# Emieeel/auto_oo

Hardware: AMD Instinct MI355X
Metric: OO-VQE energy+grad evals/sec (formaldimine CAS(4e,3o)/cc-pVDZ); 2e-transform fp64 TFLOP/s vs roofline (higher is better)
Workload: dtype f64; 1 GPU; configs[1] shape: N=43 AOs, n_occ=6, CAS(4e,3o), UCCD n_theta=4, n_kappa=327; one step = one batched call evaluating energy + full gradient of all 256 geometries of the rank (256 synthetic geometries in the job, geometry g on rank g mod n_gpus); value = evaluations/s; in-order calls on one stream; geometries_per_rank=256, batched_calls=1332, calls=in order, parallelism=geometry-sharded x1, one all_gather at the end, dist_world_size=1, devices_visible=1, device_of_rank0=0

## Files before the change

### auto_oo_amd/csrc/cas.hip

```cpp
#include "plan.h"
#include "circuit_small.h"
#include <type_traits>
#include <stdlib.h>

namespace {

constexpr int HALF_WAVES = 8;
constexpr int TRI_REG_R = 3;
constexpr int tiles_depth(int zt) { return zt == 3 ? 4 : 8; }
constexpr int stream_depth(int zt) { return zt == 3 ? 2 : 3; }
constexpr int AUX_PLAIN = 0, AUX_NT = 2;

constexpr int SYM_FULL = 0, SYM_MIRROR = 1, SYM_PACKED = 2;
__device__ __forceinline__ void tri_decode(long t, int N, int& p, int& q)
{
    const double b = 2.0 * N + 1.0;
    int pp = (int)((b - sqrt(b * b - 8.0 * (double)t)) * 0.5);
    pp = pp < 0 ? 0 : (pp > N - 1 ? N - 1 : pp);
    while (pp > 0 && (long)pp * (2 * N - pp + 1) / 2 > t) --pp;
    while (pp < N - 1 && (long)(pp + 1) * (2 * N - pp) / 2 <= t) ++pp;
    p = pp;
    q = pp + (int)(t - (long)pp * (2 * N - pp + 1) / 2);
}

// ... 2312 lines not shown
                      const int32_t* __restrict__ kap_row, const int32_t* __restrict__ kap_col,
                      int n_kappa, double* __restrict__ c0, double* __restrict__ E,
                      double* __restrict__ gvec, double* __restrict__ dE, double* __restrict__ fock,
                      double* __restrict__ gmat, const double* __restrict__ nuc_arr,
                      size_t out_stride)
{
    const int tid = threadIdx.x;
    {
        const size_t gi = blockIdx.x;
        Fcol += gi * (size_t)nrdm * M * N;
        Epart += gi * (size_t)nrdm * N;
        Cpart += gi * (size_t)N;
        c0 += gi * out_stride;
        E += gi * out_stride;
        gvec += gi * out_stride;
        if (dE) dE += gi * out_stride;
        if (fock) fock += gi * (size_t)N * N;
        if (gmat) gmat += gi * (size_t)N * N;
        if (nuc_arr) nuc = nuc_arr[gi];
    }
    for (long base = 0; base < (long)nrdm * n_kappa; base += 4 * 512) {
        int rr[4], cc[4], kk[4];
#pragma unroll
        for (int u = 0; u < 4; ++u) {
            const long idx = base + u * 512 + tid;
            const bool ok = idx < (long)nrdm * n_kappa;
            const long ii = ok ? idx : 0;
            kk[u] = (int)(ii / n_kappa);
            const int t = (int)(ii - (long)kk[u] * n_kappa);
            rr[u] = kap_row[t];
            cc[u] = kap_col[t];
        }
        double frc[4], fcr[4];
#pragma unroll
        for (int u = 0; u < 4; ++u) {
            const double* F = Fcol + (size_t)kk[u] * M * N;
            const int r = rr[u], c = cc[u];
            frc[u] = F[(size_t)(r < M ? r : 0) * N + c] * (r < M ? 1.0 : 0.0);
            fcr[u] = F[(size_t)(c < M ? c : 0) * N + r] * (c < M ? 1.0 : 0.0);
        }
#pragma unroll
        for (int u = 0; u < 4; ++u) {
            const long idx = base + u * 512 + tid;
            if (idx < (long)nrdm * n_kappa) gvec[idx] = 2.0 * (frc[u] - fcr[u]);
        }
    }
    if (fock)
        for (int idx = tid; idx < N * N; idx += 512) {
            const int m = idx / N;
            fock[idx] = m < M ? Fcol[idx] : 0.0;
        }
    if (gmat)
        for (int idx = tid; idx < N * N; idx += 512) {
            const int m = idx / N, n = idx - m * N;
            const double fmn = m < M ? Fcol[(size_t)m * N + n] : 0.0;
            const double fnm = n < M ? Fcol[(size_t)n * N + m] : 0.0;
            gmat[idx] = 2.0 * (fmn - fnm);
        }
    if (tid < nrdm) {
        const int k = tid;
        double acc = 0.0;
        for (int n = 0; n < M; ++n) acc += Epart[(size_t)k * N + n];
        if (k == 0) {
            double core = nuc;
            for (int n = 0; n < M; ++n) core += Cpart[n];
            c0[0] = core;
            E[0] = core + acc;
        } else if (dE) {
            dE[k - 1] = acc;
        }
    }
}

constexpr int TAIL_THREADS = 512;

__host__ __device__ inline bool tail_needed(int x, int y, int z, int no)
{
    const int lo = y < z ? y : z, hi = y < z ? z : y;
    if (lo >= no) return true;
    if (hi < no) return lo == hi || x == lo || x == hi;
    return x >= no || x == lo;
}

template <int KS>
__global__ __launch_bounds__(TAIL_THREADS, 2)
void cas_tail_kernel(const double* __restrict__ J, const double* __restrict__ C, const double* __restrict__ Wpre,
                     const double* __restrict__ gamma, const double* __restrict__ Gamma, int nrdm, int N, int no,
                     int na, int NC, double nuc, const double* __restrict__ nuc_arr,
                     const int32_t* __restrict__ kap_row, const int32_t* __restrict__ kap_col, int n_kappa,
                     double* __restrict__ c0, double* __restrict__ E, double* __restrict__ gvec,
                     double* __restrict__ dE, double* __restrict__ c1, double* __restrict__ c2, size_t out_stride)
{
    extern __shared__ double lds[];
    constexpr int NW = TAIL_THREADS / 64;
    constexpr int PW = (4 * KS + NW - 1) / NW;
    constexpr int PB = PW * KS > 48 ? (PW + 1) / 2 : PW;
    const int M = no + na, M2 = M * M, M3 = M2 * M;
    const int na2 = na * na, na3 = na2 * na, na4 = na2 * na2;
    const int ncol = M * (M + 1) / 2, nty = (ncol + 15) / 16;
    const long tri = (long)N * (N + 1) / 2;
    const int by = blockIdx.x;
    const int tid = threadIdx.x, lane = tid & 63;
    const int wave = __builtin_amdgcn_readfirstlane(tid >> 6);
    const int lq = lane >> 4, lr = lane & 15;
    {
        const size_t gi = by;
        J += gi * nty * tri * 16;
        C += gi * (size_t)N * N;
        Wpre += gi * (size_t)N * N;
        gamma += gi * (size_t)nrdm * na2;
        Gamma += gi * (size_t)nrdm * na4;
        c0 += gi * out_stride;
        E += gi * out_stride;
        gvec += gi * out_stride;
        if (dE) dE += gi * out_stride;
        c1 += gi * out_stride;
        c2 += gi * out_stride;
        if (nuc_arr) nuc = nuc_arr[gi];
    }
    double* Gc = lds;
    double* Cl = Gc + (size_t)N * NC;
    double* hn = Cl + (size_t)N * M;
    double* FIn = hn + (size_t)N * M;
    double* gml = FIn + (size_t)N * M;
    double* Gml = gml + (size_t)nrdm * na2;
    double* Cp = Gml + (size_t)nrdm * na4;
    int* tab = reinterpret_cast<int*>(Cp + N);
    int* wcnt = tab + M3;
    int* krow = wcnt + NW;
    int* kcol = krow + n_kappa;
    double* scr = Cp + N + (M3 + NW + 2 * n_kappa + 1) / 2;
    const int LDP = M * 16 + 8;

    typedef unsigned v2u __attribute__((ext_vector_type(2)));
    const __amdgpu_buffer_rsrc_t csrd = __builtin_amdgcn_make_buffer_rsrc(
        const_cast<double*>(C), 0, (int)((size_t)N * N * sizeof(double)), 0x00020000);
    double af[KS];
#pragma unroll
    for (int ks = 0; ks < KS; ++ks) {
        const int q = 4 * ks + lq;
        const v2u v = __builtin_amdgcn_raw_buffer_load_b64(
            csrd, (q < N && lr < M) ? (unsigned)((q * N + lr) * (int)sizeof(double)) : 0x7fffffffu, 0, 0);
        af[ks] = __builtin_bit_cast(double, v);
    }
    auto load_half = [&](double (&bf)[PB][KS], int ty, int h0) {
        const __amdgpu_buffer_rsrc_t jsrd = __builtin_amdgcn_make_buffer_rsrc(
            const_cast<double*>(J + (size_t)ty * tri * 16), 0, (int)(tri * 16 * sizeof(double)), 0x00020000);
#pragma unroll
        for (int i = 0; i < PB; ++i) {
            const int p = wave + NW * (h0 + i);
            const int pc = p < N ? p : N - 1;
            const int basep = pc * (2 * N - pc + 1) / 2 - pc;
#pragma unroll
            for (int ks = 0; ks < KS; ++ks) {
                const int q = 4 * ks + lq < N ? 4 * ks + lq : N - 1;
                const int t = q < pc ? q * (2 * N - q + 1) / 2 - q + pc : basep + q;
                const v2u v = __builtin_amdgcn_raw_buffer_load_b64(
                    jsrd, (unsigned)((t * 16 + lr) * (int)sizeof(double)), 0, 0);
                bf[i][ks] = __builtin_bit_cast(double, v);
            }
        }
    };
    double* T3s = scr;
    auto mfma_half = [&](const double (&bf)[PB][KS], int h0) {
#pragma unroll
        for (int i = 0; i < PB; ++i) {
            if (h0 + i >= PW) continue;
            const int p = wave + NW * (h0 + i);
            d4 acc = d4{0.0, 0.0, 0.0, 0.0};
#pragma unroll
            for (int ks = 0; ks < KS; ++ks) acc = mfma_f64(af[ks], bf[i][ks], acc);
            double* row = T3s + (size_t)(p < 4 * KS ? p : 0) * LDP + lr;
#pragma unroll
            for (int j = 0; j < 4; ++j) {
                const int x = lq + 4 * j;
                if (x < M && p < 4 * KS) row[x * 16] = p < N ? acc[j] : 0.0;
            }
        }
    };
    static_assert(2 * PB >= PW, "two halves cover the rows of a wave");
    double bf[PB][KS];
    load_half(bf, 0, 0);

    for (int idx = tid; idx < N * M; idx += TAIL_THREADS) {
        const int q = idx / M, x = idx - q * M;
        Cl[idx] = C[(size_t)q * N + x];
    }
    for (int idx = tid; idx < N * N; idx += TAIL_THREADS) scr[idx] = Wpre[idx];
    for (int idx = tid; idx < nrdm * na2; idx += TAIL_THREADS) gml[idx] = gamma[idx];
    for (int idx = tid; idx < nrdm * na4; idx += TAIL_THREADS) Gml[idx] = Gamma[idx];
    for (int idx = tid; idx < n_kappa; idx += TAIL_THREADS) {
        krow[idx] = kap_row[idx];
        kcol[idx] = kap_col[idx];
    }
    {
        const int total = M * ncol;
        int base = 0;
        for (int i0 = 0; i0 < total; i0 += TAIL_THREADS) {
            const int i = i0 + tid;
            int x = 0, y = 0, z = 0;
            bool need = false;
            if (i < total) {
                x = i / ncol;
                tri_decode(i - x * ncol, M, y, z);
                need = tail_needed(x, y, z, no);
            }
            const unsigned long long mask = __ballot(need);
            const int below = __popcll(mask & ((1ull << lane) - 1ull));
            if (lane == 0) wcnt[wave] = __popcll(mask);
            __syncthreads();
            int pre = base, all = 0;
            for (int w = 0; w < NW; ++w) {
                const int c = wcnt[w];
                if (w < wave) pre += c;
                all += c;
            }
            if (i < total) {
                const int v = need ? pre + below : -1;
                tab[(x * M + y) * M + z] = v;
                tab[(x * M + z) * M + y] = v;
            }
            __syncthreads();
            base += all;
        }
    }
    for (int idx = tid; idx < N * M; idx += TAIL_THREADS) {
        const int n = idx / M, x = idx - n * M;
        double acc = 0.0;
        for (int q = 0; q < N; ++q) acc += scr[(size_t)n * N + q] * Cl[q * M + x];
        hn[idx] = acc;
    }
    __syncthreads();

    {
        const int ntn = (N + 15) / 16;
        for (int ty = 0; ty < nty; ++ty) {
            mfma_half(bf, 0);
            if (PB < PW) {
                load_half(bf, ty, PB);
                mfma_half(bf, PB);
            }
            __syncthreads();
            const int yz = 16 * ty + lr;
            int off = 0;
            if (yz < ncol) {
                int y, z;
                tri_decode(yz, M, y, z);
                off = y * M + z;
            }
            int cur_nt = -1;
            double cf[KS];
            for (int tile = wave; tile < ntn * M; tile += NW) {
                const int nt = tile / M, x = tile - nt * M;
                if (nt != cur_nt) {
                    const int n = 16 * nt + lr;
#pragma unroll
                    for (int ks = 0; ks < KS; ++ks) {
                        const int pp = 4 * ks + lq;
                        const v2u v = __builtin_amdgcn_raw_buffer_load_b64(
                            csrd, (pp < N && n < N) ? (unsigned)((pp * N + n) * (int)sizeof(double)) : 0x7fffffffu,
                            0, 0);
                        cf[ks] = __builtin_bit_cast(double, v);
                    }
                    cur_nt = nt;
                }
                double tf[KS];
#pragma unroll
                for (int ks = 0; ks < KS; ++ks) tf[ks] = T3s[(size_t)(4 * ks + lq) * LDP + x * 16 + lr];
                d4 acc = d4{0.0, 0.0, 0.0, 0.0};
#pragma unroll
                for (int ks = 0; ks < KS; ++ks) acc = mfma_f64(cf[ks], tf[ks], acc);
                const int ci = yz < ncol ? tab[x * M2 + off] : -1;
                if (ci >= 0) {
#pragma unroll
                    for (int j = 0; j < 4; ++j) {
                        const int n = 16 * nt + lq + 4 * j;
                        if (n < N) Gc[(size_t)n * NC + ci] = acc[j];
                    }
                }
            }
            if (ty + 1 < nty) load_half(bf, ty + 1, 0);
            __syncthreads();
        }
    }

#define TAIL_G(n, a, b, c) Gc[(size_t)(n) * NC + tab[((a) * M + (b)) * M + (c)]]
    for (int idx = tid; idx < N * M; idx += TAIL_THREADS) {
        const int n = idx / M, x = idx - n * M;
        double fi = hn[idx];
        for (int i = 0; i < no; ++i) fi += 2.0 * TAIL_G(n, x, i, i) - TAIL_G(n, i, i, x);
        FIn[idx] = fi;
    }
    double* Fl = scr;
    double* El = Fl + (size_t)nrdm * M * N;
    double* Ga = El + (size_t)nrdm * N;
    double* Dc = Ga + (size_t)N * na3;
    for (int idx = tid; idx < N * na3; idx += TAIL_THREADS) {
        const int n = idx / na3, r = idx - n * na3;
        const int w = r / na2, x = (r / na) % na, y = r % na;
        Ga[idx] = TAIL_G(n, no + w, no + x, no + y);
    }
    for (int idx = tid; idx < N * no * na2; idx += TAIL_THREADS) {
        const int n = idx / (no * na2), r = idx - n * (no * na2);
        const int m = r / na2, v = (r / na) % na, w = r % na;
        const int V = no + v, W = no + w;
        Dc[idx] = TAIL_G(n, m, V, W) - 0.5 * TAIL_G(n, W, V, m);
    }
    __syncthreads();
    for (int n = tid; n < N; n += TAIL_THREADS) Cp[n] = n < no ? hn[n * M + n] + FIn[n * M + n] : 0.0;
    for (int idx = tid; idx < na * (na + na3); idx += TAIL_THREADS) {
        const int pl = idx / (na + na3), r0 = idx - pl * (na + na3);
        const int n = no + pl;
        if (r0 < na) {
            c1[pl * na + r0] = FIn[n * M + no + r0];
        } else {
            int t = r0 - na;
            const int i3 = t;
            const int s = t % na; t /= na;
            const int r = t % na; t /= na;
            const int q = t;
            c2[(size_t)pl * na3 + i3] = 0.5 * TAIL_G(n, no + q, no + r, no + s);
        }
    }
    const int ncore = N * nrdm * no;
    for (int idx = tid; idx < N * nrdm * M; idx += TAIL_THREADS) {
        int n, k, m;
        if (idx < ncore) {
            n = idx / (nrdm * no);
            const int r0 = idx - n * (nrdm * no);
            k = r0 / no;
            m = r0 - k * no;
        } else {
            const int j = idx - ncore;
            n = j / (nrdm * na);
            const int r0 = j - n * (nrdm * na);
            k = r0 / na;
            m = no + r0 - k * na;
        }
        const double* FIv = FIn + (size_t)n * M;
        const double* gam = gml + (size_t)k * na2;
        double val;
        if (m < no) {
            const double* Dm = Dc + ((size_t)n * no + m) * na2;
            double fa = 0.0;
            for (int v = 0; v < na; ++v)
                for (int w = 0; w < na; ++w) fa += gam[v * na + w] * Dm[v * na + w];
            val = 2.0 * ((k == 0 ? FIv[m] : 0.0) + fa);
        } else {
            const int v = m - no;
            const double* Gv = Gml + (size_t)k * na4 + (size_t)v * na3;
            double acc = 0.0;
            for (int w = 0; w < na; ++w) acc += FIv[no + w] * gam[v * na + w];
            for (int w = 0; w < na; ++w)
                for (int x = 0; x < na; ++x)
                    for (int y = 0; y < na; ++y)
                        acc += Gv[(w * na + x) * na + y] * Ga[(size_t)n * na3 + (w * na + x) * na + y];
            val = acc;
        }
        Fl[((size_t)k * M + m) * N + n] = val;
    }
    for (int idx = tid; idx < N * nrdm; idx += TAIL_THREADS) {
        const int n = idx / nrdm, k = idx - n * nrdm;
        double acc = 0.0;
        if (n >= no && n < M) {
            const int p = n - no;
            const double* FIv = FIn + (size_t)n * M;
            const double* gam = gml + (size_t)k * na2 + (size_t)p * na;
            const double* Gpq = Gml + (size_t)k * na4 + (size_t)p * na3;
            for (int q = 0; q < na; ++q) acc += FIv[no + q] * gam[q];
            for (int q = 0; q < na; ++q)
                for (int r = 0; r < na; ++r)
                    for (int s2 = 0; s2 < na; ++s2)
                        acc += 0.5 * Ga[(size_t)n * na3 + (q * na + r) * na + s2] * Gpq[(q * na + r) * na + s2];
        }
        El[(size_t)k * N + n] = acc;
    }
#undef TAIL_G
    __syncthreads();

    for (int idx = tid; idx < nrdm * n_kappa; idx += TAIL_THREADS) {
        const int k = idx / n_kappa, t = idx - k * n_kappa;
        const int r = krow[t], c = kcol[t];
        const double* F = Fl + (size_t)k * M * N;
        const double frc = F[(size_t)(r < M ? r : 0) * N + c] * (r < M ? 1.0 : 0.0);
        const double fcr = F[(size_t)(c < M ? c : 0) * N + r] * (c < M ? 1.0 : 0.0);
        gvec[idx] = 2.0 * (frc - fcr);
    }
    if (tid < nrdm) {
        const int k = tid;
        double acc = 0.0;
        for (int n = 0; n < M; ++n) acc += El[(size_t)k * N + n];
        if (k == 0) {
            double core = nuc;
            for (int n = 0; n < M; ++n) core += Cp[n];
            c0[0] = core;
            E[0] = core + acc;
        } else if (dE) {
            dE[k - 1] = acc;
        }
    }
}

}

#define OOVQE_STAGE1_DISPATCH(v, LAUNCH, ...)                                                     \
    switch ((v).kch) {                                                                            \
    case 4: LAUNCH(4, 1, 2, ##__VA_ARGS__); break;                                                \
    case 8: LAUNCH(8, 2, 5, ##__VA_ARGS__); break;                                                \
    case 11: LAUNCH(11, 3, 8, ##__VA_ARGS__); break;                                              \
    default: LAUNCH(12, 3, 10, ##__VA_ARGS__); break;                                             \
    }
#define OOVQE_KS_DISPATCH(v, LAUNCH)                                                              \
    switch ((v).ks) {                                                                             \
    case 4: LAUNCH(4); break;                                                                     \
    case 8: LAUNCH(8); break;                                                                     \
    default: LAUNCH(12); break;                                                                   \
    }

static int stage1_variant(int N, Stage1Variant* v)
{
    static const Stage1Variant rows[] = {{4, 1, 2, 4}, {8, 2, 5, 8}, {11, 3, 8, 12}, {12, 3, 10, 12}};
    for (const Stage1Variant& r : rows)
        if (N >= 1 && (N + 3) / 4 <= r.kch) {
            *v = r;
            return 0;
        }
    oovqe_set_error("cas_eval: no stage-1 kernel variant for N=%d", N);
    return OOVQE_ERR_ARG;
}

static size_t half_lds_bytes(int N, int M)
{
    const int ZT = (M + 15) / 16, nrb = (N + 15) / 16, LDM = 16 * (ZT | 1);
    return (((size_t)nrb * 16 * LDM + 511) / 512) * 512 * sizeof(double);
}
static size_t half_lds_bytes_rs(int N, int M) { return half_lds_bytes(N, M) + (size_t)HALF_WAVES * 16 * 17 * sizeof(double); }

static int stage1_half(int N, int M, int sym, bool rs, bool tiles, Stage1* s)
{
    memset(s, 0, sizeof(*s));
    OOVQE_REQUIRE(N >= 1 && M >= 1 && M <= N, "cas_half_transform: bad N=%d M=%d", N, M);
    const int ZT = (M + 15) / 16, nrb = (N + 15) / 16, ksteps = (N + 3) / 4;
    OOVQE_REQUIRE(ZT <= 3, "cas_half_transform: n_occ+ncas = %d > 48 not supported", M);
    OOVQE_REQUIRE(half_lds_bytes(N, M) <= 160 * 1024, "cas_half_transform: N=%d M=%d needs %zu B of LDS", N, M,
                  half_lds_bytes(N, M));
    s->zt = ZT;
    s->sym = sym;
    if (nrb <= 3) {
        s->kernel = S1_HALF;
        if (int rc = stage1_variant(N, &s->v)) return rc;
        snprintf(s->name, sizeof(s->name), "half_transform_kernel<%d,%d,%d>%s", ZT, s->v.kch, s->v.nrb,
                 sym ? " (slabs p <= q)" : "");
        return 0;
    }
    int waste = 1 << 30;
    for (int k = 16; k >= 10; --k) {
        const int w = (ksteps + k - 1) / k * k - ksteps;
        if (w < waste) { waste = w; s->skch = k; }
    }
    s->rs = rs && half_lds_bytes_rs(N, M) <= 160 * 1024;
    if (tiles && s->rs && sym == SYM_MIRROR) {
        s->kernel = S1_TILES;
        snprintf(s->name, sizeof(s->name), "half_tiles_kernel<%d,%d>", ZT, tiles_depth(ZT));
    } else {
        s->kernel = S1_STREAM;
        snprintf(s->name, sizeof(s->name), "half_stream_kernel<%d,%d,%d,%s>", ZT, s->skch, stream_depth(ZT), s->rs ? "true" : "false");
    }
    return 0;
}

static int half_transform_batched(const double* g_ao, const double* C, int N, int M, double* T2, int batch,
                                  oovqe_stream_t stream, const Stage1& s, double* Vk_tri = nullptr,
                                  const double* g_tiles = nullptr)
{
    OOVQE_REQUIRE(g_ao && C && T2, "cas_half_transform: null pointer");
    OOVQE_REQUIRE(!Vk_tri || (s.sym == SYM_MIRROR && N <= 48),
                  "cas_half_transform: the quarter-transformed output needs p<->q symmetric integrals and N <= 48");
    OOVQE_REQUIRE(batch >= 1 && batch <= 65535, "cas_half_transform: batch=%d", batch);
    OOVQE_REQUIRE(s.kernel != S1_TILES || g_tiles, "cas_half_transform: no tile-packed integrals");
    hipStream_t st = (hipStream_t)stream;
    const int ZT = s.zt, sym = s.sym;
    const int nrb = (N + 15) / 16;
    const long nslabs = sym == SYM_FULL ? (long)N * N : (long)N * (N + 1) / 2;
    const long want = (nslabs + HALF_WAVES - 1) / HALF_WAVES;
    oovqe_note_stage1("%s", s.name);
    oovqe_profile_mark_start(st);
// ... 113 lines not shown
    hipStream_t st = (hipStream_t)stream;
    if (N > 48) {
        for (int gi = 0; gi < batch; ++gi) {
            int rc = oovqe_eri_symmetry_flags(g_ao + (size_t)gi * N * N * N * N, N, 1, eri_flags + gi, stream);
            if (rc) return rc;
        }
        return packed ? oovqe_eri_pack(g_ao, N, batch, packed, stream) : 0;
    }
    int* flag = nullptr;
    OOVQE_CHECK_HIP(hipMalloc(&flag, sizeof(int) * (size_t)batch), "eri_ingest");
    hipError_t e = hipMemsetAsync(flag, 0, sizeof(int) * (size_t)batch, st);
    if (e == hipSuccess) {
        hipLaunchKernelGGL(eri_ingest_kernel, dim3((unsigned)(N * (N + 1) / 2), batch), dim3(256), 0, st,
                           reinterpret_cast<const unsigned long long*>(g_ao), packed, N, eri_slab_pitch(N), flag);
        e = hipGetLastError();
    }
    int* bad = (int*)malloc(sizeof(int) * (size_t)batch);
    if (!bad) e = hipErrorOutOfMemory;
    if (e == hipSuccess) e = hipMemcpyAsync(bad, flag, sizeof(int) * (size_t)batch, hipMemcpyDeviceToHost, st);
    if (e == hipSuccess) e = hipStreamSynchronize(st);
    (void)hipFree(flag);
    if (e == hipSuccess)
        for (int gi = 0; gi < batch; ++gi)
            eri_flags[gi] = ((bad[gi] & 1) ? 0u : OOVQE_ERI_PQ_SYMMETRIC) | ((bad[gi] & 2) ? 0u : OOVQE_ERI_RS_SYMMETRIC);
    free(bad);
    OOVQE_CHECK_HIP(e, "eri_ingest");
    return 0;
}

static int sym_q_contract_batched(const double* J, const double* C, double* T3, int N, int M, int batch,
                                  hipStream_t st)
{
    OOVQE_REQUIRE(M >= 1 && M <= 16 && N >= 1 && N <= 48, "sym_q_contract: N=%d M=%d", N, M);
    Stage1Variant v;
    if (int rc = stage1_variant(N, &v)) return rc;
    const unsigned threads = (unsigned)((M * M + 15) / 16 * 64);
    oovqe_profile_mark_start_l(st, LABEL_Q_TO_X);
#define OOVQE_LAUNCH_Q(KS_) \
    hipLaunchKernelGGL(sym_q_contract_kernel<KS_>, dim3(N, batch), dim3(threads), 0, st, J, C, T3, N, M)
    OOVQE_KS_DISPATCH(v, OOVQE_LAUNCH_Q)
#undef OOVQE_LAUNCH_Q
    oovqe_profile_mark_stop(st);
    OOVQE_CHECK_LAUNCH("cas_eval/sym_q_contract");
    return 0;
}

static int sym_gm_batched(const double* J, const double* C, double* Gm, int N, int M, int batch,
                          hipStream_t st, const oovqe_circuit_job_t* cj, bool packed)
{
    OOVQE_REQUIRE(M >= 1 && M <= 16 && N >= 1 && N <= 48, "sym_gm: N=%d M=%d", N, M);
    Stage1Variant v;
    if (int rc = stage1_variant(N, &v)) return rc;
    size_t lds_bytes = (size_t)4 * v.ks * (M * 16 + 8) * sizeof(double);
    if (cj && cj->lds_bytes > lds_bytes) lds_bytes = cj->lds_bytes;
    const unsigned nty = (unsigned)(((packed ? M * (M + 1) / 2 : M * M) + 15) / 16);
    oovqe_circuit_job_t job;
    memset(&job, 0, sizeof(job));
    if (cj) job = *cj;
    const unsigned nx = nty + (cj ? 1 : 0);
    const bool xcd_grid = batch > 1 && oovqe_opt(OOVQE_OPT_GM_PLAIN_GRID) == 0;
    const dim3 grid = xcd_grid ? dim3(nx * (unsigned)((batch + 7) / 8 * 8)) : dim3(nx, batch);
#define OOVQE_LAUNCH_GM2(KS_, WPE_)                                                               \
    do {                                                                                          \
        if (int rc_ = oovqe_ensure_dynamic_lds((const void*)sym_gm_kernel<KS_, WPE_>, lds_bytes)) return rc_; \
        hipLaunchKernelGGL((sym_gm_kernel<KS_, WPE_>), grid, dim3(SMALL_THREADS), lds_bytes, st,  \
                           J, C, Gm, N, M, packed ? 1 : 0, job, cj ? 1 : 0, batch);               \
    } while (0)
    const bool multi_round = ((long)nx * batch > (long)oovqe_cu_count() || oovqe_opt(OOVQE_OPT_GM_TWO_PER_CU)) &&
                             2 * lds_bytes <= 160 * 1024 && oovqe_opt(OOVQE_OPT_GM_ONE_PER_CU) == 0;
#define OOVQE_LAUNCH_GM(KS_)                                                                      \
    do {                                                                                          \
        if (multi_round) OOVQE_LAUNCH_GM2(KS_, 4);                                                \
        else OOVQE_LAUNCH_GM2(KS_, 2);                                                            \
    } while (0)
    oovqe_profile_mark_start_l(st, LABEL_P_TO_N);
    OOVQE_KS_DISPATCH(v, OOVQE_LAUNCH_GM)
    oovqe_profile_mark_stop(st);
#undef OOVQE_LAUNCH_GM
#undef OOVQE_LAUNCH_GM2
    OOVQE_CHECK_LAUNCH("cas_eval/sym_gm");
    return 0;
}

static size_t tail_lds_bytes(int N, int no, int na, int nrdm, int n_kappa, int* NC)
{
    const int M = no + na, M3 = M * M * M;
    Stage1Variant v;
    if (N > 48 || M > 16 || stage1_variant(N, &v)) return 0;
    int nc = 0;
    for (int x = 0; x < M; ++x)
        for (int y = 0; y < M; ++y)
            for (int z = y; z < M; ++z) nc += tail_needed(x, y, z, no) ? 1 : 0;
    *NC = nc;
    const size_t na2 = (size_t)na * na, na4 = na2 * na2;
    size_t scr = (size_t)N * N;
    const size_t t3 = (size_t)4 * v.ks * (M * 16 + 8);
    const size_t fe = (size_t)nrdm * M * N + (size_t)nrdm * N +
                      (size_t)N * na * na * na + (size_t)N * no * na2;
    if (t3 > scr) scr = t3;
    if (fe > scr) scr = fe;
    const size_t doubles = (size_t)N * nc + 3 * (size_t)N * M + (size_t)nrdm * (na2 + na4) + N +
                           ((size_t)M3 + TAIL_THREADS / 64 + 2 * (size_t)n_kappa + 1) / 2 + scr;
    const size_t bytes = doubles * sizeof(double);
    return bytes <= 160 * 1024 ? bytes : 0;
}

static int cas_tail_batched(const CasEvalArgs& a, const EvalPlan& p, const double* J, const double* Wpre, hipStream_t st)
{
    Stage1Variant v;
    if (int rc = stage1_variant(a.N, &v)) return rc;
#define OOVQE_LAUNCH_TAIL(KS_)                                                                    \
    do {                                                                                          \
        if (int rc_ = oovqe_ensure_dynamic_lds((const void*)cas_tail_kernel<KS_>, p.tail_lds)) return rc_; \
        hipLaunchKernelGGL((cas_tail_kernel<KS_>), dim3(a.batch), dim3(TAIL_THREADS), p.tail_lds, st, J, a.C, Wpre, \
                           a.gamma, a.Gamma, a.nrdm, a.N, a.n_occ, a.ncas, p.tail_nc, a.nuc, a.nuc_arr, a.kap_row, \
                           a.kap_col, a.n_kappa, a.out.c0, a.out.E, a.out.gvec, a.out.dE, a.out.c1, a.out.c2,       \
                           a.out_stride);                                                         \
    } while (0)
    oovqe_profile_mark_start_l(st, LABEL_P_TO_N);
    OOVQE_KS_DISPATCH(v, OOVQE_LAUNCH_TAIL)
    oovqe_profile_mark_stop(st);
#undef OOVQE_LAUNCH_TAIL
    OOVQE_CHECK_LAUNCH("cas_eval/tail");
    return 0;
}

static bool fused_plan(int N, int M, int batch, int n_cu, long chunks_opt, FusedPlan* fp)
{
    if (M > 16 || N > 48 || N < 1) return false;
    const long m2 = (long)M * M, m3 = m2 * M;
    if (chunks_opt <= 0 && (long)batch * N * N < 48L * n_cu) return false;
    long target = n_cu / batch;
    long nchunk0 = chunks_opt > 0 ? chunks_opt : target / N;
    if (nchunk0 < 1) nchunk0 = 1;
    const long cap = (2L * N * m2 - m3) / (m3 + N);
    if (cap < 1) return false;
    if (nchunk0 > cap) nchunk0 = cap;
    int qc = N, nchunk = 1;
    if (nchunk0 > 1) {
        qc = 4 * (int)((N + 4 * nchunk0 - 1) / (4 * nchunk0));
        nchunk = (N + qc - 1) / qc;
    }
    const int QR = (qc + 3) & ~3, CR = (nchunk - 1) * qc + QR;
    int ldb = (int)((m2 + 15) / 16 * 16);
    if (ldb % 32 == 0) ldb += 16;
    const size_t fixed = ((size_t)CR * 16 + 64 + 8) * sizeof(double);
    const size_t block = (size_t)QR * ldb * sizeof(double);
    const size_t task_stage = (size_t)m3 * sizeof(double);
    const long Tg = (long)nchunk * N;
    long wpg = target < 1 ? 1 : target;
    if (wpg > Tg) wpg = Tg;
    const size_t lds_cap = 160 * 1024;
    if (fixed + 2 * block + task_stage > lds_cap) return false;
    const long max_tasks = (long)((lds_cap - fixed - 2 * block) / task_stage);
    if ((Tg + wpg - 1) / wpg > max_tasks) wpg = (Tg + max_tasks - 1) / max_tasks;
    const long ntask = (Tg + wpg - 1) / wpg;
    long nbuf = (long)((lds_cap - fixed - (size_t)ntask * task_stage) / block);
    if (nbuf > 3) nbuf = 3;
    fp->nchunk = nchunk;
    fp->qc = qc;
    fp->nbuf = (int)nbuf;
    fp->ldb = ldb;
    fp->wpg = (int)wpg;
    fp->lds_bytes = fixed + (size_t)nbuf * block + (size_t)ntask * task_stage;
    return true;
}

static int half_transform_fused_batched(const double* g_ao, const double* C, int N, int M, double* T3,
                                        double* Cdup, const FusedPlan& fp, const Stage1& s, int batch, hipStream_t st)
{
#define OOVQE_LAUNCH_FUSED(KC_, NS_, NPC_)                                                        \
    do {                                                                                          \
        if (int rc_lds = oovqe_ensure_dynamic_lds((const void*)half_transform_fused_kernel<KC_, NS_>, 160 * 1024)) return rc_lds; \
        hipLaunchKernelGGL((half_transform_fused_kernel<KC_, NS_>), dim3(fp.wpg, batch),          \
                           dim3(HALF_WAVES * 64), fp.lds_bytes, st, g_ao, C, T3, Cdup, N, M,      \
                           fp.nchunk, fp.qc, fp.nbuf, fp.ldb);                                    \
    } while (0)
    oovqe_note_stage1("%s", s.name);
    oovqe_profile_mark_start(st);
    OOVQE_STAGE1_DISPATCH(s.v, OOVQE_LAUNCH_FUSED)
    oovqe_profile_mark_stop(st);
#undef OOVQE_LAUNCH_FUSED
    OOVQE_CHECK_LAUNCH("cas_eval/half_transform_fused");
    return 0;
}

static unsigned eri_slab_packed_elems(int N) { return eri_slab_pitch(N); }

extern "C" int64_t oovqe_eri_packed_size(int N)
{
    if (N < 1) return 0;
    if (N > 48) {
        const int64_t nst = (N + 15) / 16;
        return (int64_t)N * (N + 1) / 2 * (nst * (nst + 1) / 2) * 256;
    }
    return (int64_t)N * (N + 1) / 2 * eri_slab_packed_elems(N);
}

extern "C" int oovqe_eri_pack(const double* g_ao, int N, int batch, double* packed, oovqe_stream_t stream)
{
    OOVQE_REQUIRE(g_ao && packed, "eri_pack: null pointer");
    OOVQE_REQUIRE(N >= 1 && N <= 4096 && batch >= 1 && batch <= 65535, "eri_pack: N=%d batch=%d", N, batch);
    if (N > 48) {
// ... 669 lines not shown
        oovqe_profile_mark_stop(st);
        if (c.rdm_event) {
            OOVQE_CHECK_HIP(hipEventRecord(c.rdm_event, st), "oo_eval: hipEventRecord");
            c.rdm_event = nullptr;
        }
    }
    return cas_eval_batched(c, p);
}

int oovqe_half_transform_batched_impl(const double* g_ao, const double* C, int N, int M, double* T2,
                                      int batch, unsigned eri_flags, oovqe_stream_t stream, double* Vk_tri)
{
    const bool pq = (eri_flags & OOVQE_ERI_PQ_SYMMETRIC) != 0;
    const bool rs = (eri_flags & OOVQE_ERI_RS_SYMMETRIC) != 0 && oovqe_opt(OOVQE_OPT_SYM_NO_RS) == 0;
    Stage1 s;
    if (int rc = stage1_half(N, M, pq ? SYM_MIRROR : SYM_FULL, rs, false, &s)) return rc;
    return half_transform_batched(g_ao, C, N, M, T2, batch, stream, s, Vk_tri);
}

extern "C" int oovqe_oo_eval_batch(const double* theta, int n_theta, const oovqe_gate_t* gates,
                                   int n_gates, int n_qubits, uint32_t init_index, const double* g_ao,
                                   const double* h_ao, const double* C, const double* nuc, int N,
                                   int n_occ, int ncas, const int32_t* kap_row, const int32_t* kap_col,
                                   int n_kappa, int derivatives, int batch, double* work, double* out,
                                   unsigned eri_flags, const double* g_packed, oovqe_stream_t stream)
{
    OOVQE_REQUIRE(nuc, "oo_eval_batch: null nuc");
    return oovqe_oo_eval_batched_impl(OoEvalArgs{
        .theta = theta, .n_theta = n_theta, .gates = gates, .n_gates = n_gates, .n_qubits = n_qubits,
        .init_index = init_index, .derivatives = derivatives, .work = work, .out = out,
        .cas = {.g_ao = g_ao, .h_ao = h_ao, .C = C, .nuc_arr = nuc, .N = N, .n_occ = n_occ, .ncas = ncas,
                .kap_row = kap_row, .kap_col = kap_col, .n_kappa = n_kappa, .batch = batch, .stream = stream,
                .eri_flags = eri_flags, .g_packed = g_packed}});
}

extern "C" int oovqe_oo_eval(const double* theta, int n_theta, const oovqe_gate_t* gates, int n_gates,
                             int n_qubits, uint32_t init_index, const double* g_ao,
                             const double* h_ao, const double* C, double nuc, int N, int n_occ,
                             int ncas, const int32_t* kap_row, const int32_t* kap_col, int n_kappa,
                             int derivatives, double* work, double* out, unsigned eri_flags,
                             oovqe_stream_t stream)
{
    return oovqe_oo_eval_batched_impl(OoEvalArgs{
        .theta = theta, .n_theta = n_theta, .gates = gates, .n_gates = n_gates, .n_qubits = n_qubits,
        .init_index = init_index, .derivatives = derivatives, .work = work, .out = out,
        .cas = {.g_ao = g_ao, .h_ao = h_ao, .C = C, .nuc = nuc, .N = N, .n_occ = n_occ, .ncas = ncas,
                .kap_row = kap_row, .kap_col = kap_col, .n_kappa = n_kappa, .batch = 1, .stream = stream,
                .eri_flags = eri_flags}});
}

extern "C" const char* oovqe_oo_eval_plan_describe(int n_theta, int n_gates, int n_qubits, int N, int n_occ,
                                                   int ncas, int n_kappa, int derivatives, int batch,
                                                   unsigned eri_flags, int have_packed)
{
    static thread_local char line[512];
    static const char* const path_names[] = {"packed_tail", "packed_split", "packed_two_step", "fused", "column", "staged"};
    static const char* const circuit_names[] = {"none", "rides", "own"};
    static const char* const block_names[WB_COUNT] = {"Jp", "T3", "Gmw", "Cdup", "T2", "U", "Fcol", "Epart", "Cpart"};
    const EvalShape s{.N = N, .n_occ = n_occ, .ncas = ncas, .nrdm = derivatives ? 1 + n_theta : 1, .n_kappa = n_kappa,
                      .batch = batch, .eri_flags = eri_flags, .packed = have_packed != 0, .n_qubits = n_qubits,
                      .n_gates = n_gates, .n_cu = oovqe_cu_count(), .opt = oovqe_eval_opts()};
    EvalPlan p;
    if (n_qubits != 0 && n_qubits != 2 * ncas) {
        oovqe_set_error("oo_eval: n_qubits != 2*ncas");
        return nullptr;
    }
    if (oovqe_eval_plan(s, &p)) return nullptr;
    const bool k1 = p.path == PATH_PACKED_TWO_STEP || p.path == PATH_FUSED || p.path == PATH_COLUMN;
    const long M = n_occ + ncas, K = p.path == PATH_FUSED ? (long)p.fused.nchunk * N : N;
    const int hosts = k1 && oovqe_contract_hosts_circuit(1, (int)K, N, p.path == PATH_COLUMN ? N * M * M : M * M * M, 0, batch, s.opt.k1);
    size_t n = 0;
    auto add = [&](const char* fmt, auto... args) {
        if (n < sizeof(line)) n += (size_t)snprintf(line + n, sizeof(line) - n, fmt, args...);
    };
    add("path=%s; stage1=%s; circuit=%s; w=%d; launches=%ld; k1_hosts=%d; labels=", path_names[p.path], p.stage1.name,
        circuit_names[p.circuit], p.w ? 1 : 0, p.launches, hosts);
    for (int l = 0; l < LABEL_COUNT; ++l) add("%s%d", l ? "," : "", p.labels[l]);
    add("%s", "; blocks=");
    for (int b = 0, first = 1; b < WB_COUNT; ++b)
        if (p.len[b]) {
            add("%s%s@%zu+%zu", first ? "" : ",", block_names[b], p.off[b], p.len[b]);
            first = 0;
        }
    return line;
}

__global__ void fock_core_active_kernel(const double* __restrict__ h, const double* __restrict__ g,
                                        const double* __restrict__ gam, int N, int no, int na,
                                        double* __restrict__ FI, double* __restrict__ FA)
{
    const int idx = blockIdx.x * blockDim.x + threadIdx.x;
    if (idx >= N * N) return;
    const int m = idx / N, n = idx - m * N;
    const size_t n2 = (size_t)N * N, n3 = n2 * N;
    const double* gm = g + (size_t)m * n3;
    if (FI) {
        double acc = h[idx];
        for (int i = 0; i < no; ++i)
            acc += 2.0 * gm[(size_t)n * n2 + (size_t)i * N + i] - gm[(size_t)i * n2 + (size_t)i * N + n];
        FI[idx] = acc;
    }
    if (FA) {
        double acc = 0.0;
        for (int v = 0; v < na; ++v)
            for (int w = 0; w < na; ++w) {
                const int V = no + v, W = no + w;
                acc += gam[v * na + w] * (gm[(size_t)n * n2 + (size_t)V * N + W] -
                                          0.5 * gm[(size_t)W * n2 + (size_t)V * N + n]);
            }
        FA[idx] = acc;
    }
}

extern "C" int oovqe_fock_core_active(const double* h_mo, const double* g_mo, const double* gamma, int N,
                                      int n_occ, int ncas, double* fock_core, double* fock_active,
                                      oovqe_stream_t stream)
{
    OOVQE_REQUIRE(g_mo && (fock_core || fock_active), "fock_core_active: null pointer");
    OOVQE_REQUIRE(!fock_core || h_mo, "fock_core_active: h_mo required for fock_core");
    OOVQE_REQUIRE(!fock_active || gamma, "fock_core_active: gamma required for fock_active");
    OOVQE_REQUIRE(N >= 1 && n_occ >= 0 && ncas >= 1 && n_occ + ncas <= N, "fock_core_active: sizes");
    hipLaunchKernelGGL(fock_core_active_kernel, dim3((N * N + 255) / 256), dim3(256), 0,
                       (hipStream_t)stream, h_mo, g_mo, gamma, N, n_occ, ncas, fock_core, fock_active);
    OOVQE_CHECK_LAUNCH("fock_core_active");
    return 0;
}
```

Measured before the change: 575,700 evals/s.

## Pipeline J loads in the CAS tail kernel and keep C tiles in registers

Reworks the J half-transform loop in cas_tail_kernel. J row groups are now double-buffered and prefetched across tiles, with scheduling barriers placed between the MFMA and load phases. The C second-transform operands are preloaded once into registers instead of being reloaded per tile, and the first-step A operand is read from LDS. A new KS=11 specialization is selected for N=41..44, which trims the K depth for N=43. Optional wall-clock probe marks are added behind a compile flag. The trade-off is higher register pressure, which could spill or lower occupancy.

New measurement: 621,900 evals/s, median of 6. +8.0%, better.

```diff
diff --git a/auto_oo_amd/csrc/cas.hip b/auto_oo_amd/csrc/cas.hip
--- a/auto_oo_amd/csrc/cas.hip
+++ b/auto_oo_amd/csrc/cas.hip
@@ -2418,6 +2418,19 @@
     return x >= no || x == lo;
 }
 
+#ifdef OOVQE_TAIL_PROBE
+constexpr int TAIL_PROBE_WGS = 512, TAIL_PROBE_MARKS = 32;
+__device__ long long g_tail_probe[TAIL_PROBE_WGS][TAIL_PROBE_MARKS];
+#define TAIL_MARK(i)                                                                              \
+    do {                                                                                          \
+        __syncthreads();                                                                          \
+        if (threadIdx.x == 0 && blockIdx.x < TAIL_PROBE_WGS && (i) < TAIL_PROBE_MARKS)            \
+            g_tail_probe[blockIdx.x][i] = wall_clock64();                                         \
+    } while (0)
+#else
+#define TAIL_MARK(i) do {} while (0)
+#endif
+
 template <int KS>
 __global__ __launch_bounds__(TAIL_THREADS, 2)
 void cas_tail_kernel(const double* __restrict__ J, const double* __restrict__ C, const double* __restrict__ Wpre,
@@ -2430,7 +2443,8 @@
     extern __shared__ double lds[];
     constexpr int NW = TAIL_THREADS / 64;
     constexpr int PW = (4 * KS + NW - 1) / NW;
-    constexpr int PB = PW * KS > 48 ? (PW + 1) / 2 : PW;
+    constexpr int GR = 2, NG = (PW + GR - 1) / GR;
+    constexpr int NTN = (4 * KS + 15) / 16;
     const int M = no + na, M2 = M * M, M3 = M2 * M;
     const int na2 = na * na, na3 = na2 * na, na4 = na2 * na2;
     const int ncol = M * (M + 1) / 2, nty = (ncol + 15) / 16;
@@ -2471,52 +2485,80 @@
     typedef unsigned v2u __attribute__((ext_vector_type(2)));
     const __amdgpu_buffer_rsrc_t csrd = __builtin_amdgcn_make_buffer_rsrc(
         const_cast<double*>(C), 0, (int)((size_t)N * N * sizeof(double)), 0x00020000);
-    double af[KS];
+    double cfa[NTN][KS];
+#pragma unroll
+    for (int nt = 0; nt < NTN; ++nt)
+#pragma unroll
+        for (int ks = 0; ks < KS; ++ks) {
+            const int pp = 4 * ks + lq, n = 16 * nt + lr;
+            const v2u v = __builtin_amdgcn_raw_buffer_load_b64(
+                csrd, (pp < N && n < N) ? (unsigned)((pp * N + n) * (int)sizeof(double)) : 0x7fffffffu, 0, 0);
+            cfa[nt][ks] = __builtin_bit_cast(double, v);
+        }
+    constexpr bool COLQ_REGS = KS < 12;
+    int colq[KS];
 #pragma unroll
     for (int ks = 0; ks < KS; ++ks) {
-        const int q = 4 * ks + lq;
-        const v2u v = __builtin_amdgcn_raw_buffer_load_b64(
-            csrd, (q < N && lr < M) ? (unsigned)((q * N + lr) * (int)sizeof(double)) : 0x7fffffffu, 0, 0);
-        af[ks] = __builtin_bit_cast(double, v);
-    }
-    auto load_half = [&](double (&bf)[PB][KS], int ty, int h0) {
-        const __amdgpu_buffer_rsrc_t jsrd = __builtin_amdgcn_make_buffer_rsrc(
-            const_cast<double*>(J + (size_t)ty * tri * 16), 0, (int)(tri * 16 * sizeof(double)), 0x00020000);
-#pragma unroll
-        for (int i = 0; i < PB; ++i) {
-            const int p = wave + NW * (h0 + i);
-            const int pc = p < N ? p : N - 1;
-            const int basep = pc * (2 * N - pc + 1) / 2 - pc;
+        const int q = 4 * ks + lq < N ? 4 * ks + lq : N - 1;
+        colq[ks] = ((q * (2 * N - q + 1) / 2 - q) * 16 + lr) * (int)sizeof(double);
+    }
+    const int lin0 = (lq * 16 + lr) * (int)sizeof(double);
+    auto load_group = [&](double (&bf)[GR][KS], int ty, int g) {
+#pragma unroll
+        for (int r = 0; r < GR; ++r) {
+            const int i = g * GR + r;
+            if (i >= PW) continue;
+            int wv = wave;
+#if defined(__HIP_DEVICE_COMPILE__)
+            asm volatile("" : "+s"(wv));
+#endif
+            const int p = wv + NW * i;
+            int lqo = lq;
+#if defined(__HIP_DEVICE_COMPILE__)
+            asm volatile("" : "+v"(lqo));
+#endif
+            const __amdgpu_buffer_rsrc_t jsrd = __builtin_amdgcn_make_buffer_rsrc(
+                const_cast<double*>(J + (size_t)(ty < nty ? ty : 0) * tri * 16), 0,
+                p < N && ty < nty ? (int)(tri * 16 * sizeof(double)) : 0, 0x00020000);
+            const int colp = p * 16 * (int)sizeof(double);
+            const int rowp = (p * (2 * N - p + 1) / 2 - p) * 16 * (int)sizeof(double) + lin0;
 #pragma unroll
             for (int ks = 0; ks < KS; ++ks) {
-                const int q = 4 * ks + lq < N ? 4 * ks + lq : N - 1;
-                const int t = q < pc ? q * (2 * N - q + 1) / 2 - q + pc : basep + q;
-                const v2u v = __builtin_amdgcn_raw_buffer_load_b64(
-                    jsrd, (unsigned)((t * 16 + lr) * (int)sizeof(double)), 0, 0);
-                bf[i][ks] = __builtin_bit_cast(double, v);
+                const int q = 4 * ks + lqo;
+                const int cq = COLQ_REGS ? colq[ks] : (q * (2 * N - 1 - q) / 2 * 16 + lr) * (int)sizeof(double);
+                const int off = lq < p - 4 * ks ? cq + colp : rowp + ks * 64 * (int)sizeof(double);
+                const v2u v = __builtin_amdgcn_raw_buffer_load_b64(jsrd, (unsigned)off, 0, 0);
+                bf[r][ks] = __builtin_bit_cast(double, v);
             }
         }
     };
     double* T3s = scr;
-    auto mfma_half = [&](const double (&bf)[PB][KS], int h0) {
-#pragma unroll
-        for (int i = 0; i < PB; ++i) {
-            if (h0 + i >= PW) continue;
-            const int p = wave + NW * (h0 + i);
+    auto mfma_group = [&](const double (&af)[KS], const double (&bf)[GR][KS], int g) {
+#pragma unroll
+        for (int r = 0; r < GR; ++r) {
+            const int i = g * GR + r;
+            if (i >= PW) continue;
+            int wv = wave;
+#if defined(__HIP_DEVICE_COMPILE__)
+            asm volatile("" : "+s"(wv));
+#endif
+            const int p = wv + NW * i;
+            if (p >= 4 * KS) continue;
             d4 acc = d4{0.0, 0.0, 0.0, 0.0};
-#pragma unroll
-            for (int ks = 0; ks < KS; ++ks) acc = mfma_f64(af[ks], bf[i][ks], acc);
-            double* row = T3s + (size_t)(p < 4 * KS ? p : 0) * LDP + lr;
-#pragma unroll
-            for (int j = 0; j < 4; ++j) {
-                const int x = lq + 4 * j;
-                if (x < M && p < 4 * KS) row[x * 16] = p < N ? acc[j] : 0.0;
-            }
+            if (p < N) {
+#pragma unroll
+                for (int ks = 0; ks < KS; ++ks) acc = mfma_f64(af[ks], bf[r][ks], acc);
+            }
+            double* row = T3s + (p * LDP + lq * 16 + lr);
+#pragma unroll
+            for (int j = 0; j < 4; ++j)
+                if (lq + 4 * j < M) row[j * 64] = acc[j];
         }
     };
-    static_assert(2 * PB >= PW, "two halves cover the rows of a wave");
-    double bf[PB][KS];
-    load_half(bf, 0, 0);
+    double bs[2][GR][KS];
+    TAIL_MARK(0);
+#pragma unroll
+    for (int s0 = 0; s0 < 2; ++s0) load_group(bs[s0], s0 / NG, s0 % NG);
 
     for (int idx = tid; idx < N * M; idx += TAIL_THREADS) {
         const int q = idx / M, x = idx - q * M;
@@ -2529,6 +2571,7 @@
         krow[idx] = kap_row[idx];
         kcol[idx] = kap_col[idx];
     }
+    TAIL_MARK(1);
     {
         const int total = M * ncol;
         int base = 0;
@@ -2560,6 +2603,7 @@
             base += all;
         }
     }
+    TAIL_MARK(2);
     for (int idx = tid; idx < N * M; idx += TAIL_THREADS) {
         const int n = idx / M, x = idx - n * M;
         double acc = 0.0;
@@ -2567,16 +2611,33 @@
         hn[idx] = acc;
     }
     __syncthreads();
+    TAIL_MARK(3);
 
     {
         const int ntn = (N + 15) / 16;
-        for (int ty = 0; ty < nty; ++ty) {
-            mfma_half(bf, 0);
-            if (PB < PW) {
-                load_half(bf, ty, PB);
-                mfma_half(bf, PB);
+        auto tail_tile = [&](auto par, int ty) {
+            constexpr int P = decltype(par)::value;
+            double af[KS];
+            int lqv = lq;
+#if defined(__HIP_DEVICE_COMPILE__)
+            asm volatile("" : "+v"(lqv));
+#endif
+#pragma unroll
+            for (int ks = 0; ks < KS; ++ks) {
+                const int q = 4 * ks + lqv;
+                const double c = Cl[(q < N ? q : N - 1) * M + (lr < M ? lr : 0)];
+                af[ks] = (q < N && lr < M) ? c : 0.0;
+            }
+#pragma unroll
+            for (int g = 0; g < NG; ++g) {
+                mfma_group(af, bs[(P + g) & 1], g);
+                __builtin_amdgcn_sched_barrier(0);
+                load_group(bs[(P + g) & 1], ty + (g + 2) / NG, (g + 2) % NG);
+                __builtin_amdgcn_sched_barrier(0);
+                if (g == 0) TAIL_MARK(ty < 3 ? 4 + 3 * ty : 31);
             }
             __syncthreads();
+            TAIL_MARK(ty < 3 ? 5 + 3 * ty : 31);
             const int yz = 16 * ty + lr;
             int off = 0;
             if (yz < ncol) {
@@ -2584,39 +2645,34 @@
                 tri_decode(yz, M, y, z);
                 off = y * M + z;
             }
-            int cur_nt = -1;
-            double cf[KS];
-            for (int tile = wave; tile < ntn * M; tile += NW) {
-                const int nt = tile / M, x = tile - nt * M;
-                if (nt != cur_nt) {
-                    const int n = 16 * nt + lr;
-#pragma unroll
-                    for (int ks = 0; ks < KS; ++ks) {
-                        const int pp = 4 * ks + lq;
-                        const v2u v = __builtin_amdgcn_raw_buffer_load_b64(
-                            csrd, (pp < N && n < N) ? (unsigned)((pp * N + n) * (int)sizeof(double)) : 0x7fffffffu,
-                            0, 0);
-                        cf[ks] = __builtin_bit_cast(double, v);
-                    }
-                    cur_nt = nt;
-                }
-                double tf[KS];
-#pragma unroll
-                for (int ks = 0; ks < KS; ++ks) tf[ks] = T3s[(size_t)(4 * ks + lq) * LDP + x * 16 + lr];
-                d4 acc = d4{0.0, 0.0, 0.0, 0.0};
-#pragma unroll
-                for (int ks = 0; ks < KS; ++ks) acc = mfma_f64(cf[ks], tf[ks], acc);
-                const int ci = yz < ncol ? tab[x * M2 + off] : -1;
-                if (ci >= 0) {
-#pragma unroll
-                    for (int j = 0; j < 4; ++j) {
-                        const int n = 16 * nt + lq + 4 * j;
-                        if (n < N) Gc[(size_t)n * NC + ci] = acc[j];
+#pragma unroll
+            for (int nt = 0; nt < NTN; ++nt) {
+                if (nt >= ntn) continue;
+                const int t0 = nt * M;
+                for (int tile = t0 + (wave - t0 % NW + NW) % NW; tile < t0 + M; tile += NW) {
+                    const int x = tile - t0;
+                    double tf[KS];
+#pragma unroll
+                    for (int ks = 0; ks < KS; ++ks) tf[ks] = T3s[(size_t)(4 * ks + lq) * LDP + x * 16 + lr];
+                    d4 acc = d4{0.0, 0.0, 0.0, 0.0};
+#pragma unroll
+                    for (int ks = 0; ks < KS; ++ks) acc = mfma_f64(cfa[nt][ks], tf[ks], acc);
+                    const int ci = yz < ncol ? tab[x * M2 + off] : -1;
+                    if (ci >= 0) {
+#pragma unroll
+                        for (int j = 0; j < 4; ++j) {
+                            const int n = 16 * nt + lq + 4 * j;
+                            if (n < N) Gc[(size_t)n * NC + ci] = acc[j];
+                        }
                     }
                 }
             }
-            if (ty + 1 < nty) load_half(bf, ty + 1, 0);
             __syncthreads();
+            TAIL_MARK(ty < 3 ? 6 + 3 * ty : 31);
+        };
+        for (int ty = 0; ty < nty; ty += 2) {
+            tail_tile(std::integral_constant<int, 0>{}, ty);
+            if (ty + 1 < nty) tail_tile(std::integral_constant<int, NG & 1>{}, ty + 1);
         }
     }
 
@@ -2627,6 +2683,7 @@
         for (int i = 0; i < no; ++i) fi += 2.0 * TAIL_G(n, x, i, i) - TAIL_G(n, i, i, x);
         FIn[idx] = fi;
     }
+    TAIL_MARK(13);
     double* Fl = scr;
     double* El = Fl + (size_t)nrdm * M * N;
     double* Ga = El + (size_t)nrdm * N;
@@ -2643,6 +2700,7 @@
         Dc[idx] = TAIL_G(n, m, V, W) - 0.5 * TAIL_G(n, W, V, m);
     }
     __syncthreads();
+    TAIL_MARK(14);
     for (int n = tid; n < N; n += TAIL_THREADS) Cp[n] = n < no ? hn[n * M + n] + FIn[n * M + n] : 0.0;
     for (int idx = tid; idx < na * (na + na3); idx += TAIL_THREADS) {
         const int pl = idx / (na + na3), r0 = idx - pl * (na + na3);
@@ -2658,6 +2716,7 @@
             c2[(size_t)pl * na3 + i3] = 0.5 * TAIL_G(n, no + q, no + r, no + s);
         }
     }
+    TAIL_MARK(15);
     const int ncore = N * nrdm * no;
     for (int idx = tid; idx < N * nrdm * M; idx += TAIL_THREADS) {
         int n, k, m;
@@ -2695,6 +2754,7 @@
         }
         Fl[((size_t)k * M + m) * N + n] = val;
     }
+    TAIL_MARK(16);
     for (int idx = tid; idx < N * nrdm; idx += TAIL_THREADS) {
         const int n = idx / nrdm, k = idx - n * nrdm;
         double acc = 0.0;
@@ -2713,6 +2773,7 @@
     }
 #undef TAIL_G
     __syncthreads();
+    TAIL_MARK(17);
 
     for (int idx = tid; idx < nrdm * n_kappa; idx += TAIL_THREADS) {
         const int k = idx / n_kappa, t = idx - k * n_kappa;
@@ -2735,9 +2796,18 @@
             dE[k - 1] = acc;
         }
     }
-}
-
-}
+    TAIL_MARK(18);
+}
+
+}
+
+#ifdef OOVQE_TAIL_PROBE
+extern "C" int oovqe_tail_probe_read(long long* out, int n)
+{
+    const size_t bytes = sizeof(long long) * (size_t)(n < TAIL_PROBE_WGS * TAIL_PROBE_MARKS ? n : TAIL_PROBE_WGS * TAIL_PROBE_MARKS);
+    return hipMemcpyFromSymbol(out, HIP_SYMBOL(g_tail_probe), bytes) == hipSuccess ? 0 : 1;
+}
+#endif
 
 #define OOVQE_STAGE1_DISPATCH(v, LAUNCH, ...)                                                     \
     switch ((v).kch) {                                                                            \
@@ -3017,6 +3087,15 @@
     return 0;
 }
 
+static int tail_depth(int N, const Stage1Variant& v) { return N >= 41 && N <= 44 ? 11 : v.ks; }
+#define OOVQE_TAIL_DISPATCH(ks, LAUNCH)                                                           \
+    switch (ks) {                                                                                 \
+    case 4: LAUNCH(4); break;                                                                     \
+    case 8: LAUNCH(8); break;                                                                     \
+    case 11: LAUNCH(11); break;                                                                   \
+    default: LAUNCH(12); break;                                                                   \
+    }
+
 static size_t tail_lds_bytes(int N, int no, int na, int nrdm, int n_kappa, int* NC)
 {
     const int M = no + na, M3 = M * M * M;
@@ -3029,7 +3108,7 @@
     *NC = nc;
     const size_t na2 = (size_t)na * na, na4 = na2 * na2;
     size_t scr = (size_t)N * N;
-    const size_t t3 = (size_t)4 * v.ks * (M * 16 + 8);
+    const size_t t3 = (size_t)4 * tail_depth(N, v) * (M * 16 + 8);
     const size_t fe = (size_t)nrdm * M * N + (size_t)nrdm * N +
                       (size_t)N * na * na * na + (size_t)N * no * na2;
     if (t3 > scr) scr = t3;
@@ -3053,7 +3132,7 @@
                            a.out_stride);                                                         \
     } while (0)
     oovqe_profile_mark_start_l(st, LABEL_P_TO_N);
-    OOVQE_KS_DISPATCH(v, OOVQE_LAUNCH_TAIL)
+    OOVQE_TAIL_DISPATCH(tail_depth(a.N, v), OOVQE_LAUNCH_TAIL)
     oovqe_profile_mark_stop(st);
 #undef OOVQE_LAUNCH_TAIL
     OOVQE_CHECK_LAUNCH("cas_eval/tail");
@@ -3889,6 +3968,11 @@
             add("%s%s@%zu+%zu", first ? "" : ",", block_names[b], p.off[b], p.len[b]);
             first = 0;
         }
+    if (p.path == PATH_PACKED_TAIL) {
+        Stage1Variant v;
+        if (stage1_variant(N, &v)) return nullptr;
+        add("; tail=cas_tail_kernel<%d>; tail_lds=%zu", tail_depth(N, v), p.tail_lds);
+    }
     return line;
 }
 
```
